# r9y9/deepvoice3_pytorch

Measured on NVIDIA H100. Metric: mel-frames/sec training step (B=16,T_mel=800), higher is better.
Workload: dtype f32 via split 16-bit pairs (fp16 pairs forward, bf16 pairs for gradients; 3 wgmma passes per product, fp32 accumulate)

## Files before the change

### deepvoice3_pytorch_b200/csrc/tc_common.cuh

```cuda
#pragma once
#include <cuda.h>
#include <cuda_bf16.h>
#include "common.cuh"

namespace dv3 {
namespace tc {

__device__ __forceinline__ uint32_t smem_u32(const void* p) { return (uint32_t)__cvta_generic_to_shared(p); }

__device__ __forceinline__ void mbar_init(uint64_t* bar, uint32_t count) {
    asm volatile("mbarrier.init.shared::cta.b64 [%0], %1;" ::"r"(smem_u32(bar)), "r"(count));
}
__device__ __forceinline__ void fence_barrier_init() {
    asm volatile("fence.mbarrier_init.release.cluster;" ::: "memory");
}
__device__ __forceinline__ void fence_proxy_async() {
    asm volatile("fence.proxy.async.shared::cta;" ::: "memory");
}
__device__ __forceinline__ void mbar_arrive_expect_tx(uint64_t* bar, uint32_t bytes) {
    asm volatile("mbarrier.arrive.expect_tx.shared::cta.b64 _, [%0], %1;" ::"r"(smem_u32(bar)), "r"(bytes)
                 : "memory");
}
__device__ __forceinline__ void mbar_arrive(uint64_t* bar) {
    asm volatile("mbarrier.arrive.shared::cta.b64 _, [%0];" ::"r"(smem_u32(bar)) : "memory");
}
__device__ __forceinline__ void mbar_wait(uint64_t* bar, uint32_t parity) {
    asm volatile(
        "{\n"
        ".reg .pred p;\n"
        "DV3_WAIT:\n"
        "mbarrier.try_wait.parity.shared::cta.b64 p, [%0], %1;\n"
        "@p bra DV3_DONE;\n"
        "bra DV3_WAIT;\n"
        "DV3_DONE:\n"
        "}\n" ::"r"(smem_u32(bar)),
        "r"(parity)
        : "memory");
}

__device__ __forceinline__ void tma_load_3d(void* smem_dst, const CUtensorMap* map, uint64_t* bar, int c0, int c1,
                                            int c2) {
    asm volatile(
        "cp.async.bulk.tensor.3d.shared::cluster.global.mbarrier::complete_tx::bytes [%0], [%1, {%3, %4, %5}], [%2];"
        ::"r"(smem_u32(smem_dst)), "l"(map), "r"(smem_u32(bar)), "r"(c0), "r"(c1), "r"(c2)
        : "memory");
}
__device__ __forceinline__ void prefetch_tmap(const CUtensorMap* map) {
    asm volatile("prefetch.tensormap [%0];" ::"l"(map) : "memory");
}
__device__ __forceinline__ void prefetch_l2(const void* p) {
    asm volatile("prefetch.global.L2 [%0];" ::"l"(p));
}
__device__ __forceinline__ void tma_store_3d(const CUtensorMap* map, const void* smem_src, int c0, int c1, int c2) {
    asm volatile("cp.async.bulk.tensor.3d.global.shared::cta.bulk_group [%0, {%2, %3, %4}], [%1];"
                 ::"l"(map), "r"(smem_u32(smem_src)), "r"(c0), "r"(c1), "r"(c2)
                 : "memory");
}
__device__ __forceinline__ void bulk_commit() { asm volatile("cp.async.bulk.commit_group;" ::: "memory"); }
__device__ __forceinline__ void bulk_wait_read() { asm volatile("cp.async.bulk.wait_group.read 0;" ::: "memory"); }
__device__ __forceinline__ void bulk_wait() { asm volatile("cp.async.bulk.wait_group 0;" ::: "memory"); }
__device__ __forceinline__ void mbar_arrive_cnt(uint64_t* bar, uint32_t count) {
    asm volatile("mbarrier.arrive.shared::cta.b64 _, [%0], %1;" ::"r"(smem_u32(bar)), "r"(count) : "memory");
}
__device__ __forceinline__ void named_bar_sync(int id, int threads) {
    asm volatile("bar.sync %0, %1;" ::"r"(id), "r"(threads) : "memory");
}

template <int N>
__device__ __forceinline__ void setmaxnreg_dec() { asm volatile("setmaxnreg.dec.sync.aligned.u32 %0;" ::"n"(N)); }
template <int N>
__device__ __forceinline__ void setmaxnreg_inc() { asm volatile("setmaxnreg.inc.sync.aligned.u32 %0;" ::"n"(N)); }

__device__ __forceinline__ void wgmma_fence() { asm volatile("wgmma.fence.sync.aligned;" ::: "memory"); }
__device__ __forceinline__ void wgmma_commit() { asm volatile("wgmma.commit_group.sync.aligned;" ::: "memory"); }
template <int N>
__device__ __forceinline__ void wgmma_wait() { asm volatile("wgmma.wait_group.sync.aligned %0;" ::"n"(N) : "memory"); }
__device__ __forceinline__ int frag_row(int i, int warp_in_wg, int lane) {
    return 16 * warp_in_wg + (lane >> 2) + 8 * ((i >> 1) & 1);
}
__device__ __forceinline__ int frag_col(int i, int lane) { return 8 * (i >> 2) + 2 * (lane & 3) + (i & 1); }

__device__ __forceinline__ uint64_t make_wgmma_desc(uint32_t saddr, uint32_t lbo, uint32_t sbo, uint32_t layout) {
    uint64_t d = 0;
    d |= (uint64_t)((saddr & 0x3FFFF) >> 4);
    d |= (uint64_t)((lbo >> 4) & 0x3FFF) << 16;
    d |= (uint64_t)((sbo >> 4) & 0x3FFF) << 32;
    d |= (uint64_t)layout << 62;
    return d;
}
constexpr uint32_t WG_SW128 = 1, WG_SW64 = 2;

template <int TA, int TB>
__device__ __forceinline__ void wgmma_f16_n64(float* d, uint64_t a, uint64_t b, uint32_t acc) {
    asm volatile(
        "{\n.reg .pred p;\nsetp.ne.b32 p, %34, 0;\n"
        "wgmma.mma_async.sync.aligned.m64n64k16.f32.f16.f16 {%0, %1, %2, %3, %4, %5, %6, %7, %8, %9, %10, %11, %12, %13, %14, %15, %16, %17, %18, %19, %20, %21, %22, %23, %24, %25, %26, %27, %28, %29, %30, %31}, %32, %33, p, 1, 1, %35, %36;\n}\n"
        : "+f"(d[0]), "+f"(d[1]), "+f"(d[2]), "+f"(d[3]), "+f"(d[4]), "+f"(d[5]), "+f"(d[6]), "+f"(d[7]), "+f"(d[8]), "+f"(d[9]), "+f"(d[10]), "+f"(d[11]), "+f"(d[12]), "+f"(d[13]), "+f"(d[14]), "+f"(d[15]), "+f"(d[16]), "+f"(d[17]), "+f"(d[18]), "+f"(d[19]), "+f"(d[20]), "+f"(d[21]), "+f"(d[22]), "+f"(d[23]), "+f"(d[24]), "+f"(d[25]), "+f"(d[26]), "+f"(d[27]), "+f"(d[28]), "+f"(d[29]), "+f"(d[30]), "+f"(d[31])
        : "l"(a), "l"(b), "r"(acc), "n"(TA), "n"(TB));
}
template <int TA, int TB>
__device__ __forceinline__ void wgmma_bf16_n64(float* d, uint64_t a, uint64_t b, uint32_t acc) {
    asm volatile(
        "{\n.reg .pred p;\nsetp.ne.b32 p, %34, 0;\n"
        "wgmma.mma_async.sync.aligned.m64n64k16.f32.bf16.bf16 {%0, %1, %2, %3, %4, %5, %6, %7, %8, %9, %10, %11, %12, %13, %14, %15, %16, %17, %18, %19, %20, %21, %22, %23, %24, %25, %26, %27, %28, %29, %30, %31}, %32, %33, p, 1, 1, %35, %36;\n}\n"
        : "+f"(d[0]), "+f"(d[1]), "+f"(d[2]), "+f"(d[3]), "+f"(d[4]), "+f"(d[5]), "+f"(d[6]), "+f"(d[7]), "+f"(d[8]), "+f"(d[9]), "+f"(d[10]), "+f"(d[11]), "+f"(d[12]), "+f"(d[13]), "+f"(d[14]), "+f"(d[15]), "+f"(d[16]), "+f"(d[17]), "+f"(d[18]), "+f"(d[19]), "+f"(d[20]), "+f"(d[21]), "+f"(d[22]), "+f"(d[23]), "+f"(d[24]), "+f"(d[25]), "+f"(d[26]), "+f"(d[27]), "+f"(d[28]), "+f"(d[29]), "+f"(d[30]), "+f"(d[31])
        : "l"(a), "l"(b), "r"(acc), "n"(TA), "n"(TB));
}
template <int TA, int TB>
__device__ __forceinline__ void wgmma_f16_n128(float* d, uint64_t a, uint64_t b, uint32_t acc) {
    asm volatile(
        "{\n.reg .pred p;\nsetp.ne.b32 p, %66, 0;\n"
        "wgmma.mma_async.sync.aligned.m64n128k16.f32.f16.f16 {%0, %1, %2, %3, %4, %5, %6, %7, %8, %9, %10, %11, %12, %13, %14, %15, %16, %17, %18, %19, %20, %21, %22, %23, %24, %25, %26, %27, %28, %29, %30, %31, %32, %33, %34, %35, %36, %37, %38, %39, %40, %41, %42, %43, %44, %45, %46, %47, %48, %49, %50, %51, %52, %53, %54, %55, %56, %57, %58, %59, %60, %61, %62, %63}, %64, %65, p, 1, 1, %67, %68;\n}\n"
        : "+f"(d[0]), "+f"(d[1]), "+f"(d[2]), "+f"(d[3]), "+f"(d[4]), "+f"(d[5]), "+f"(d[6]), "+f"(d[7]), "+f"(d[8]), "+f"(d[9]), "+f"(d[10]), "+f"(d[11]), "+f"(d[12]), "+f"(d[13]), "+f"(d[14]), "+f"(d[15]), "+f"(d[16]), "+f"(d[17]), "+f"(d[18]), "+f"(d[19]), "+f"(d[20]), "+f"(d[21]), "+f"(d[22]), "+f"(d[23]), "+f"(d[24]), "+f"(d[25]), "+f"(d[26]), "+f"(d[27]), "+f"(d[28]), "+f"(d[29]), "+f"(d[30]), "+f"(d[31]), "+f"(d[32]), "+f"(d[33]), "+f"(d[34]), "+f"(d[35]), "+f"(d[36]), "+f"(d[37]), "+f"(d[38]), "+f"(d[39]), "+f"(d[40]), "+f"(d[41]), "+f"(d[42]), "+f"(d[43]), "+f"(d[44]), "+f"(d[45]), "+f"(d[46]), "+f"(d[47]), "+f"(d[48]), "+f"(d[49]), "+f"(d[50]), "+f"(d[51]), "+f"(d[52]), "+f"(d[53]), "+f"(d[54]), "+f"(d[55]), "+f"(d[56]), "+f"(d[57]), "+f"(d[58]), "+f"(d[59]), "+f"(d[60]), "+f"(d[61]), "+f"(d[62]), "+f"(d[63])
        : "l"(a), "l"(b), "r"(acc), "n"(TA), "n"(TB));
}
template <int TA, int TB>
__device__ __forceinline__ void wgmma_bf16_n128(float* d, uint64_t a, uint64_t b, uint32_t acc) {
    asm volatile(
        "{\n.reg .pred p;\nsetp.ne.b32 p, %66, 0;\n"
        "wgmma.mma_async.sync.aligned.m64n128k16.f32.bf16.bf16 {%0, %1, %2, %3, %4, %5, %6, %7, %8, %9, %10, %11, %12, %13, %14, %15, %16, %17, %18, %19, %20, %21, %22, %23, %24, %25, %26, %27, %28, %29, %30, %31, %32, %33, %34, %35, %36, %37, %38, %39, %40, %41, %42, %43, %44, %45, %46, %47, %48, %49, %50, %51, %52, %53, %54, %55, %56, %57, %58, %59, %60, %61, %62, %63}, %64, %65, p, 1, 1, %67, %68;\n}\n"
        : "+f"(d[0]), "+f"(d[1]), "+f"(d[2]), "+f"(d[3]), "+f"(d[4]), "+f"(d[5]), "+f"(d[6]), "+f"(d[7]), "+f"(d[8]), "+f"(d[9]), "+f"(d[10]), "+f"(d[11]), "+f"(d[12]), "+f"(d[13]), "+f"(d[14]), "+f"(d[15]), "+f"(d[16]), "+f"(d[17]), "+f"(d[18]), "+f"(d[19]), "+f"(d[20]), "+f"(d[21]), "+f"(d[22]), "+f"(d[23]), "+f"(d[24]), "+f"(d[25]), "+f"(d[26]), "+f"(d[27]), "+f"(d[28]), "+f"(d[29]), "+f"(d[30]), "+f"(d[31]), "+f"(d[32]), "+f"(d[33]), "+f"(d[34]), "+f"(d[35]), "+f"(d[36]), "+f"(d[37]), "+f"(d[38]), "+f"(d[39]), "+f"(d[40]), "+f"(d[41]), "+f"(d[42]), "+f"(d[43]), "+f"(d[44]), "+f"(d[45]), "+f"(d[46]), "+f"(d[47]), "+f"(d[48]), "+f"(d[49]), "+f"(d[50]), "+f"(d[51]), "+f"(d[52]), "+f"(d[53]), "+f"(d[54]), "+f"(d[55]), "+f"(d[56]), "+f"(d[57]), "+f"(d[58]), "+f"(d[59]), "+f"(d[60]), "+f"(d[61]), "+f"(d[62]), "+f"(d[63])
        : "l"(a), "l"(b), "r"(acc), "n"(TA), "n"(TB));
}
template <int TA, int TB>
__device__ __forceinline__ void wgmma_f16_n256(float* d, uint64_t a, uint64_t b, uint32_t acc) {
    asm volatile(
        "{\n.reg .pred p;\nsetp.ne.b32 p, %130, 0;\n"
        "wgmma.mma_async.sync.aligned.m64n256k16.f32.f16.f16 {%0, %1, %2, %3, %4, %5, %6, %7, %8, %9, %10, %11, %12, %13, %14, %15, %16, %17, %18, %19, %20, %21, %22, %23, %24, %25, %26, %27, %28, %29, %30, %31, %32, %33, %34, %35, %36, %37, %38, %39, %40, %41, %42, %43, %44, %45, %46, %47, %48, %49, %50, %51, %52, %53, %54, %55, %56, %57, %58, %59, %60, %61, %62, %63, %64, %65, %66, %67, %68, %69, %70, %71, %72, %73, %74, %75, %76, %77, %78, %79, %80, %81, %82, %83, %84, %85, %86, %87, %88, %89, %90, %91, %92, %93, %94, %95, %96, %97, %98, %99, %100, %101, %102, %103, %104, %105, %106, %107, %108, %109, %110, %111, %112, %113, %114, %115, %116, %117, %118, %119, %120, %121, %122, %123, %124, %125, %126, %127}, %128, %129, p, 1, 1, %131, %132;\n}\n"
        : "+f"(d[0]), "+f"(d[1]), "+f"(d[2]), "+f"(d[3]), "+f"(d[4]), "+f"(d[5]), "+f"(d[6]), "+f"(d[7]), "+f"(d[8]), "+f"(d[9]), "+f"(d[10]), "+f"(d[11]), "+f"(d[12]), "+f"(d[13]), "+f"(d[14]), "+f"(d[15]), "+f"(d[16]), "+f"(d[17]), "+f"(d[18]), "+f"(d[19]), "+f"(d[20]), "+f"(d[21]), "+f"(d[22]), "+f"(d[23]), "+f"(d[24]), "+f"(d[25]), "+f"(d[26]), "+f"(d[27]), "+f"(d[28]), "+f"(d[29]), "+f"(d[30]), "+f"(d[31]), "+f"(d[32]), "+f"(d[33]), "+f"(d[34]), "+f"(d[35]), "+f"(d[36]), "+f"(d[37]), "+f"(d[38]), "+f"(d[39]), "+f"(d[40]), "+f"(d[41]), "+f"(d[42]), "+f"(d[43]), "+f"(d[44]), "+f"(d[45]), "+f"(d[46]), "+f"(d[47]), "+f"(d[48]), "+f"(d[49]), "+f"(d[50]), "+f"(d[51]), "+f"(d[52]), "+f"(d[53]), "+f"(d[54]), "+f"(d[55]), "+f"(d[56]), "+f"(d[57]), "+f"(d[58]), "+f"(d[59]), "+f"(d[60]), "+f"(d[61]), "+f"(d[62]), "+f"(d[63]), "+f"(d[64]), "+f"(d[65]), "+f"(d[66]), "+f"(d[67]), "+f"(d[68]), "+f"(d[69]), "+f"(d[70]), "+f"(d[71]), "+f"(d[72]), "+f"(d[73]), "+f"(d[74]), "+f"(d[75]), "+f"(d[76]), "+f"(d[77]), "+f"(d[78]), "+f"(d[79]), "+f"(d[80]), "+f"(d[81]), "+f"(d[82]), "+f"(d[83]), "+f"(d[84]), "+f"(d[85]), "+f"(d[86]), "+f"(d[87]), "+f"(d[88]), "+f"(d[89]), "+f"(d[90]), "+f"(d[91]), "+f"(d[92]), "+f"(d[93]), "+f"(d[94]), "+f"(d[95]), "+f"(d[96]), "+f"(d[97]), "+f"(d[98]), "+f"(d[99]), "+f"(d[100]), "+f"(d[101]), "+f"(d[102]), "+f"(d[103]), "+f"(d[104]), "+f"(d[105]), "+f"(d[106]), "+f"(d[107]), "+f"(d[108]), "+f"(d[109]), "+f"(d[110]), "+f"(d[111]), "+f"(d[112]), "+f"(d[113]), "+f"(d[114]), "+f"(d[115]), "+f"(d[116]), "+f"(d[117]), "+f"(d[118]), "+f"(d[119]), "+f"(d[120]), "+f"(d[121]), "+f"(d[122]), "+f"(d[123]), "+f"(d[124]), "+f"(d[125]), "+f"(d[126]), "+f"(d[127])
        : "l"(a), "l"(b), "r"(acc), "n"(TA), "n"(TB));
}
template <int TA, int TB>
__device__ __forceinline__ void wgmma_bf16_n256(float* d, uint64_t a, uint64_t b, uint32_t acc) {
    asm volatile(
        "{\n.reg .pred p;\nsetp.ne.b32 p, %130, 0;\n"
        "wgmma.mma_async.sync.aligned.m64n256k16.f32.bf16.bf16 {%0, %1, %2, %3, %4, %5, %6, %7, %8, %9, %10, %11, %12, %13, %14, %15, %16, %17, %18, %19, %20, %21, %22, %23, %24, %25, %26, %27, %28, %29, %30, %31, %32, %33, %34, %35, %36, %37, %38, %39, %40, %41, %42, %43, %44, %45, %46, %47, %48, %49, %50, %51, %52, %53, %54, %55, %56, %57, %58, %59, %60, %61, %62, %63, %64, %65, %66, %67, %68, %69, %70, %71, %72, %73, %74, %75, %76, %77, %78, %79, %80, %81, %82, %83, %84, %85, %86, %87, %88, %89, %90, %91, %92, %93, %94, %95, %96, %97, %98, %99, %100, %101, %102, %103, %104, %105, %106, %107, %108, %109, %110, %111, %112, %113, %114, %115, %116, %117, %118, %119, %120, %121, %122, %123, %124, %125, %126, %127}, %128, %129, p, 1, 1, %131, %132;\n}\n"
        : "+f"(d[0]), "+f"(d[1]), "+f"(d[2]), "+f"(d[3]), "+f"(d[4]), "+f"(d[5]), "+f"(d[6]), "+f"(d[7]), "+f"(d[8]), "+f"(d[9]), "+f"(d[10]), "+f"(d[11]), "+f"(d[12]), "+f"(d[13]), "+f"(d[14]), "+f"(d[15]), "+f"(d[16]), "+f"(d[17]), "+f"(d[18]), "+f"(d[19]), "+f"(d[20]), "+f"(d[21]), "+f"(d[22]), "+f"(d[23]), "+f"(d[24]), "+f"(d[25]), "+f"(d[26]), "+f"(d[27]), "+f"(d[28]), "+f"(d[29]), "+f"(d[30]), "+f"(d[31]), "+f"(d[32]), "+f"(d[33]), "+f"(d[34]), "+f"(d[35]), "+f"(d[36]), "+f"(d[37]), "+f"(d[38]), "+f"(d[39]), "+f"(d[40]), "+f"(d[41]), "+f"(d[42]), "+f"(d[43]), "+f"(d[44]), "+f"(d[45]), "+f"(d[46]), "+f"(d[47]), "+f"(d[48]), "+f"(d[49]), "+f"(d[50]), "+f"(d[51]), "+f"(d[52]), "+f"(d[53]), "+f"(d[54]), "+f"(d[55]), "+f"(d[56]), "+f"(d[57]), "+f"(d[58]), "+f"(d[59]), "+f"(d[60]), "+f"(d[61]), "+f"(d[62]), "+f"(d[63]), "+f"(d[64]), "+f"(d[65]), "+f"(d[66]), "+f"(d[67]), "+f"(d[68]), "+f"(d[69]), "+f"(d[70]), "+f"(d[71]), "+f"(d[72]), "+f"(d[73]), "+f"(d[74]), "+f"(d[75]), "+f"(d[76]), "+f"(d[77]), "+f"(d[78]), "+f"(d[79]), "+f"(d[80]), "+f"(d[81]), "+f"(d[82]), "+f"(d[83]), "+f"(d[84]), "+f"(d[85]), "+f"(d[86]), "+f"(d[87]), "+f"(d[88]), "+f"(d[89]), "+f"(d[90]), "+f"(d[91]), "+f"(d[92]), "+f"(d[93]), "+f"(d[94]), "+f"(d[95]), "+f"(d[96]), "+f"(d[97]), "+f"(d[98]), "+f"(d[99]), "+f"(d[100]), "+f"(d[101]), "+f"(d[102]), "+f"(d[103]), "+f"(d[104]), "+f"(d[105]), "+f"(d[106]), "+f"(d[107]), "+f"(d[108]), "+f"(d[109]), "+f"(d[110]), "+f"(d[111]), "+f"(d[112]), "+f"(d[113]), "+f"(d[114]), "+f"(d[115]), "+f"(d[116]), "+f"(d[117]), "+f"(d[118]), "+f"(d[119]), "+f"(d[120]), "+f"(d[121]), "+f"(d[122]), "+f"(d[123]), "+f"(d[124]), "+f"(d[125]), "+f"(d[126]), "+f"(d[127])
        : "l"(a), "l"(b), "r"(acc), "n"(TA), "n"(TB));
// ... 16 lines not shown
```

### deepvoice3_pytorch_b200/csrc/tc_gemm.cu

```cuda
#include "tc_common.cuh"
#include "tc_ring.cuh"
#include "../../include/dv3b200.h"

namespace dv3 {

using namespace tc;

constexpr int TC_CONV_THREADS = 512;
constexpr int TC_PRODUCER_REGS = 24;
constexpr int TC_CONSUMER_REGS = 168;
constexpr int TC_EPILOGUE_REGS = 152;
static_assert(TC_PRODUCER_REGS <= 65536 / TC_CONV_THREADS && TC_CONSUMER_REGS >= 65536 / TC_CONV_THREADS &&
              TC_EPILOGUE_REGS >= 65536 / TC_CONV_THREADS, "setmaxnreg direction of each warpgroup");
static_assert(128 * TC_PRODUCER_REGS + 256 * TC_CONSUMER_REGS + 128 * TC_EPILOGUE_REGS <= 65536, "register file");
constexpr int TC_EPILOGUE_LEAD = 3 * 128;
constexpr int TC_LAST_PARTS = 3;
constexpr int MAX_TAPS_TC = 8;
enum { TC_GATED = 0, TC_CONV = 1 };

struct TcMaps { CUtensorMap a[2]; CUtensorMap b[2]; };

struct TcParams {
    int T;
    int Nc;
// ... 205 lines not shown
    static_assert(Cfg::NCOLS <= 128, "main + cross accumulators must fit in the registers of a consumer thread");
    static_assert(Cfg::STAGES >= 2, "pipeline needs at least two stages");
    constexpr int STAGE = Cfg::STAGE, STAGES = Cfg::STAGES;
    constexpr int NR = Cfg::NCOLS / 2;
    pdl_trigger();
    extern __shared__ uint8_t smem_raw[];
    uint8_t* smem = smem_raw + ((1024 - (smem_u32(smem_raw) & 1023)) & 1023);
    float* acc_tile = reinterpret_cast<float*>(smem + STAGES * STAGE);
    uint64_t* full = reinterpret_cast<uint64_t*>(smem + STAGES * STAGE + Cfg::ACC_TILE + Cfg::STAGING);
    uint64_t* empty = full + STAGES;
    uint64_t* acc_full = empty + STAGES;
    uint64_t* acc_empty = acc_full + 1;
    uint64_t* in_full = acc_empty + 1;
    const int warp = threadIdx.x >> 5, lane = threadIdx.x & 31;

    if (threadIdx.x == 0) {
#pragma unroll
        for (int pl = 0; pl < NPL; ++pl) prefetch_tmap(&maps.a[pl]);
#pragma unroll
        for (int pl = 0; pl < NPL; ++pl) prefetch_tmap(&maps.b[pl]);
        for (int s = 0; s < STAGES; ++s) { mbar_init(&full[s], 1); mbar_init(&empty[s], 2); }
        mbar_init(acc_full, 256);
        mbar_init(acc_empty, 128);
        mbar_init(in_full, 1);
        fence_barrier_init();
    }
    __syncthreads();
    pdl_wait();

    if (warp >= 12) {
        setmaxnreg_inc<TC_EPILOGUE_REGS>();
        const Handoff h = {acc_tile, acc_tile + Cfg::ACC_TILE / 4, acc_empty, in_full};
        if (blockIdx.x < num_units) stage(decode(blockIdx.x), h);
        int n = 0;
        for (int u = blockIdx.x; u < num_units; u += gridDim.x, ++n) {
            const auto w = decode(u);
            const bool last = u + gridDim.x >= num_units;
            mbar_wait(acc_full, n & 1);
            if (last) epilogue(w, n, h, TC_LAST_PARTS - 1, TC_LAST_PARTS);
            else {
                epilogue(w, n, h, 0, 1);
                stage(decode(u + gridDim.x), h);
            }
        }
    } else if (warp >= 8) {
        setmaxnreg_dec<TC_PRODUCER_REGS>();
        if (warp == 8 && lane == 0) {
            int it = 0;
            for (int u = blockIdx.x; u < num_units; u += gridDim.x) {
                const auto w = decode(u);
                for (int kit = 0; kit < w.n_iters; ++kit, ++it) {
                    const int s = it % STAGES, ph = (it / STAGES) & 1;
                    mbar_wait(&empty[s], ph ^ 1);
                    mbar_arrive_expect_tx(&full[s], STAGE);
                    load(w, kit, smem + s * STAGE, &full[s]);
                }
            }
        }
    } else {
        setmaxnreg_inc<TC_CONSUMER_REGS>();
        const int wg = warp >> 2, wq = warp & 3;
        float acc[NR], xacc[NPL == 2 ? NR : 1];
        int it = 0, n = 0;
        for (int u = blockIdx.x; u < num_units; u += gridDim.x, ++n) {
            const auto w = decode(u);
#pragma unroll
            for (int i = 0; i < NR; ++i) {
                acc[i] = 0.f;
                if constexpr (NPL == 2) xacc[i] = 0.f;
            }
            for (int kit = 0; kit < w.n_iters; ++kit, ++it) {
                const int s = it % STAGES, ph = (it / STAGES) & 1;
                mbar_wait(&full[s], ph);
                wgmma_fence();
                mma(smem + s * STAGE, wg, acc, xacc);
                wgmma_commit();
                wgmma_wait<1>();
                if (kit > 0 && (threadIdx.x & 127) == 0) mbar_arrive(&empty[(it - 1) % STAGES]);
            }
            wgmma_wait<0>();
            if (w.n_iters > 0 && (threadIdx.x & 127) == 0) mbar_arrive(&empty[(it - 1) % STAGES]);
            const float gm = gmain(w);
            mbar_wait(acc_empty, (n & 1) ^ 1);
            const int sw = (((wq & 1) << 2) | (lane >> 4)) ^ ((lane & 3) << 1);
            float* const frag0 = Cfg::DENSE ? acc_tile + (2 * wg + (wq >> 1)) * Cfg::NCOLS * 32 + (lane & 3) * 64 +
                                                  ((lane >> 2) & 3)
                                            : acc_tile;
#pragma unroll
            for (int i = 0; i < NR; ++i) {
                float* dst = Cfg::DENSE
                    ? frag0 + (i >> 2) * 256 + (i & 1) * 32 + ((sw ^ (i & 3)) << 2)
                    : &acc_tile[(64 * wg + frag_row(i, wq, lane)) * Cfg::ACC_PITCH + frag_col(i, lane)];
                if constexpr (NPL == 2) *dst = fmaf(xacc[i], LO_INV, acc[i] * gm);
                else *dst = acc[i] * gm;
            }
            mbar_arrive(acc_full);
            if (u + gridDim.x >= num_units) {
                const Handoff h = {acc_tile, acc_tile + Cfg::ACC_TILE / 4, acc_empty, in_full};
                mbar_wait(acc_full, n & 1);
                epilogue(w, n, h, wg, TC_LAST_PARTS);
            }
        }
    }
}

template <int MODE, int NBOX, int BR, int BK, bool BF16, int NPL>
__global__ void __launch_bounds__(TC_CONV_THREADS, 1)
tc_conv_kernel(const __grid_constant__ TcMaps maps, const __grid_constant__ TcOutMaps om,
               const __grid_constant__ TcParams p, int tiles_x, int tiles_y, int num_tiles) {
    using Cfg = TcCfg<NBOX, BK, BR, NPL>;
    constexpr int NCOLS = Cfg::NCOLS;
    constexpr int TILE = 128 * BK * 2, TILE_B = BR * BK * 2;
    constexpr int B_OFF = NPL * TILE;
    constexpr int A_HALF = 64 * BK * 2;
    const int n_iters = p.k * p.kb_n;

    struct Tile { int a_row0, a_z, b_row0, b_row1, n_iters; };
    auto decode = [&](int tile) {
        Tile w;
        const int ty = tile % tiles_y, r = tile / tiles_y;
        w.a_z = r / tiles_x;
        w.a_row0 = (r % tiles_x) * 128;
        if (MODE == TC_GATED) { w.b_row0 = ty * BR; w.b_row1 = p.Nc + ty * BR; }
        else { w.b_row0 = ty * BR * NBOX; w.b_row1 = w.b_row0 + BR; }
        w.n_iters = n_iters;
        return w;
    };
    auto load = [&](const Tile& w, int kit, uint8_t* st, uint64_t* bar) {
        const int j = kit / p.kb_n, kb = kit - j * p.kb_n;
        const int ax = kb * BK, ay = w.a_row0 + p.tap_off[j];
        const int by0 = j * p.rows_per_tap + w.b_row0, by1 = j * p.rows_per_tap + w.b_row1;
#pragma unroll
        for (int pl = 0; pl < NPL; ++pl) {
            tma_load_3d(st + pl * TILE, &maps.a[pl], bar, ax, ay, w.a_z);
            uint8_t* bdst = st + B_OFF + pl * NBOX * TILE_B;
            tma_load_3d(bdst, &maps.b[pl], bar, ax, by0, 0);
            if (NBOX == 2) tma_load_3d(bdst + TILE_B, &maps.b[pl], bar, ax, by1, 0);
        }
    };
    auto mma = [&](const uint8_t* st, int wg, float* acc, float* xacc) {
        const uint32_t sa = smem_u32(st) + wg * A_HALF, sb = smem_u32(st + B_OFF);
#pragma unroll
        for (int kk = 0; kk < BK / 16; ++kk) {
            const uint32_t ko = kk * 32;
            const uint64_t a0 = make_desc<BK>(sa + ko), b0 = make_desc<BK>(sb + ko);
            wgmma_mma<NCOLS, 0, 0>(BF16, acc, a0, b0, 1);
            if constexpr (NPL == 2) {
                const uint64_t a1 = make_desc<BK>(sa + TILE + ko), b1 = make_desc<BK>(sb + NBOX * TILE_B + ko);
                wgmma_mma<NCOLS, 0, 0>(BF16, xacc, a0, b1, 1);
                wgmma_mma<NCOLS, 0, 0>(BF16, xacc, a1, b0, 1);
            }
        }
    };
    auto gmain = [&](const Tile&) { return p.gmain; };
    auto epilogue = [&](const Tile& w, int n, const Handoff& h, int part, int nparts) {
        if (MODE == TC_GATED) {
            if (nparts == 1) epilogue_gated<BR, 32>(p, om, h, n, w.a_row0, w.a_z, w.b_row0, 0, 1);
            else epilogue_gated<BR, BR / 8>(p, om, h, n, w.a_row0, w.a_z, w.b_row0, part, nparts);
        } else {
            if (nparts == 1) epilogue_conv<NCOLS, 32>(p, om, h, w.a_row0, w.a_z, w.b_row0, 0, 1);
            else epilogue_conv<NCOLS, NCOLS / 8>(p, om, h, w.a_row0, w.a_z, w.b_row0, part, nparts);
        }
    };
    auto stage = [&](const Tile& w, const Handoff& h) {
        if (MODE == TC_GATED) {
            stage_residual<BR>(p, om, h, w.a_row0, w.a_z, w.b_row0);
            if (p.spk) prefetch_bct(p.spk, p.T, p.Nc, w.a_z, w.b_row0, BR, w.a_row0);
        } else {
            if (p.addmode != 0) prefetch_bct(p.e1, p.T, p.Nc, w.a_z, w.b_row0, NCOLS, w.a_row0);
            if (p.addmode == 2) prefetch_bct(p.e2, p.T, p.Nc, w.a_z, w.b_row0, NCOLS, w.a_row0);
        }
    };
    tc_pipeline<Cfg, NPL>(maps, num_tiles, decode, load, mma, gmain, epilogue, stage);
}

struct TcMnParams {
    int T, B, Mw, Nw, k;
    int tap_off[MAX_TAPS_TC];
    int nsplit, batches_per_split, kb_n;
    int tiles_n, tiles_m, num_units;
    float* dw; long long split_stride;
    int msplit; long long s_m, s_mh, s_n, s_j;
    float gcoef;
};

template <int NPL>
__global__ void __launch_bounds__(TC_CONV_THREADS, 1)
tc_wgrad_mn_kernel(const __grid_constant__ TcMaps maps, const __grid_constant__ TcMnParams p) {
    using Cfg = WgCfg<NPL>;
    constexpr int A_PL = 2 * WG_BOX, B_PL = 2 * WG_BOX;
    constexpr uint32_t LBO = 4096, SBO = 1024;

    struct Unit { int m0, n0, j, s, b_beg, n_iters; };
    auto decode = [&](int u) {
        Unit w;
        w.n0 = (u % p.tiles_n) * 128;
        int r = u / p.tiles_n;
        w.m0 = (r % p.tiles_m) * 128;
        r /= p.tiles_m;
        w.j = r % p.k;
        w.s = r / p.k;
        w.b_beg = w.s * p.batches_per_split;
        const int b_end = min(p.B, w.b_beg + p.batches_per_split);
        w.n_iters = (b_end > w.b_beg ? b_end - w.b_beg : 0) * p.kb_n;
        return w;
    };
    auto load = [&](const Unit& w, int kit, uint8_t* st, uint64_t* bar) {
        const int bi = kit / p.kb_n, tc_ = kit - bi * p.kb_n;
        const int b = w.b_beg + bi, t0 = tc_ * 32;
#pragma unroll
        for (int pl = 0; pl < NPL; ++pl) {
#pragma unroll
            for (int h = 0; h < 2; ++h)
                tma_load_3d(st + pl * A_PL + h * WG_BOX, &maps.a[pl], bar, w.m0 + h * 64, t0, b);
#pragma unroll
            for (int q = 0; q < 2; ++q)
                tma_load_3d(st + NPL * A_PL + pl * B_PL + q * WG_BOX, &maps.b[pl], bar, w.n0 + q * 64,
                            t0 + p.tap_off[w.j], b);
        }
    };
    auto mma = [&](const uint8_t* st, int wg, float* acc, float* xacc) {
        const uint32_t sa = smem_u32(st);
#pragma unroll
        for (int kk = 0; kk < 2; ++kk) {
            const uint32_t ko = kk * 16 * 128;
            const uint64_t a0 = make_wgmma_desc(sa + wg * WG_BOX + ko, LBO, SBO, WG_SW128);
            const uint64_t b0 = make_wgmma_desc(sa + NPL * A_PL + ko, LBO, SBO, WG_SW128);
            wgmma_mma<128, 1, 1>(true, acc, a0, b0, 1);
            if constexpr (NPL == 2) {
                const uint64_t a1 = make_wgmma_desc(sa + A_PL + wg * WG_BOX + ko, LBO, SBO, WG_SW128);
                const uint64_t b1 = make_wgmma_desc(sa + 2 * A_PL + B_PL + ko, LBO, SBO, WG_SW128);
                wgmma_mma<128, 1, 1>(true, xacc, a0, b1, 1);
                wgmma_mma<128, 1, 1>(true, xacc, a1, b0, 1);
            }
        }
    };
    auto gmain = [&](const Unit& w) { return 1.f + p.gcoef * (float)(2 * w.n_iters); };
    auto epilogue = [&](const Unit& w, int, const Handoff& h, int part, int nparts) {
        const float* acc_tile = h.tile;
        const int r = threadIdx.x & 127;
        const int cw = nparts == 1 ? 128 : 16;
        float* __restrict__ out = p.dw + (size_t)w.s * p.split_stride + (size_t)w.j * p.s_j;
        const int rows = min(128, p.Mw - w.m0), cols = min(128, p.Nw - w.n0);
        if (p.s_n == 1) {
            if (r < cols) {
                float* __restrict__ o = out + w.n0 + r;
#pragma unroll 1
                for (int i0 = part * cw; i0 < rows; i0 += nparts * cw) {
                    const int i1 = min(i0 + cw, rows);
                    int mr = (w.m0 + i0) % p.msplit, mq = (w.m0 + i0) / p.msplit;
#pragma unroll 4
                    for (int i = i0; i < i1; ++i) {
                        o[(size_t)mr * p.s_m + (size_t)mq * p.s_mh] = acc_tile[i * Cfg::ACC_PITCH + r];
                        if (++mr == p.msplit) { mr = 0; ++mq; }
                    }
                }
            }
        } else if (r < rows) {
            const int m = w.m0 + r;
            float* __restrict__ o = out + (size_t)(m % p.msplit) * p.s_m + (size_t)(m / p.msplit) * p.s_mh +
                                    (size_t)w.n0 * p.s_n;
            const float* arow = acc_tile + r * Cfg::ACC_PITCH;
#pragma unroll 1
            for (int c0 = part * cw; c0 < cols; c0 += nparts * cw) {
                const int c1 = min(c0 + cw, cols);
#pragma unroll 4
                for (int c = c0; c < c1; ++c) o[(size_t)c * p.s_n] = arow[c];
            }
        }
        if (threadIdx.x >= TC_EPILOGUE_LEAD) mbar_arrive(h.acc_empty);
    };
    tc_pipeline<Cfg, NPL>(maps, p.num_units, decode, load, mma, gmain, epilogue, [](const Unit&, const Handoff&) {});
}

typedef CUresult (*EncodeTiledFn)(CUtensorMap*, CUtensorMapDataType, cuuint32_t, void*, const cuuint64_t*,
                                  const cuuint64_t*, const cuuint32_t*, const cuuint32_t*, CUtensorMapInterleave,
                                  CUtensorMapSwizzle, CUtensorMapL2promotion, CUtensorMapFloatOOBfill);

static EncodeTiledFn encode_fn() {
    static const EncodeTiledFn fn = [] {
        void* f = nullptr;
        cudaDriverEntryPointQueryResult qres;
        cudaError_t e = cudaGetDriverEntryPoint("cuTensorMapEncodeTiled", &f, cudaEnableDefault, &qres);
        return (e == cudaSuccess) ? (EncodeTiledFn)f : (EncodeTiledFn) nullptr;
    }();
    return fn;
}

int encode_tmap_bf16_3d(CUtensorMap* map, const void* base, uint64_t d0, uint64_t d1, uint64_t d2,
                        uint64_t stride1_bytes, uint64_t stride2_bytes, uint32_t box0, uint32_t box1) {
    const EncodeTiledFn enc = encode_fn();
    if (!enc) { set_error("cuTensorMapEncodeTiled entry point unavailable"); return 1; }
    cuuint64_t dims[3] = {d0, d1, d2};
    cuuint64_t strides[2] = {stride1_bytes, stride2_bytes};
    cuuint32_t box[3] = {box0, box1, 1};
    cuuint32_t estr[3] = {1, 1, 1};
    const CUtensorMapSwizzle sw = box0 * 2 == 128 ? CU_TENSOR_MAP_SWIZZLE_128B : CU_TENSOR_MAP_SWIZZLE_64B;
    CUresult r = enc(map, CU_TENSOR_MAP_DATA_TYPE_BFLOAT16, 3, const_cast<void*>(base), dims, strides, box, estr,
                     CU_TENSOR_MAP_INTERLEAVE_NONE, sw, CU_TENSOR_MAP_L2_PROMOTION_L2_256B,
                     CU_TENSOR_MAP_FLOAT_OOB_FILL_NONE);
    if (r != CUDA_SUCCESS) {
        set_error("cuTensorMapEncodeTiled failed (%d): dims=(%llu,%llu,%llu) strides=(%llu,%llu) box=(%u,%u)", (int)r,
                  (unsigned long long)d0, (unsigned long long)d1, (unsigned long long)d2,
                  (unsigned long long)stride1_bytes, (unsigned long long)stride2_bytes, box0, box1);
        return 1;
    }
    return 0;
}

static int encode_tmap_f32_bct(CUtensorMap* map, const float* base, int B, int Nc, int T, int box_c) {
    const EncodeTiledFn enc = encode_fn();
    if (!enc) { set_error("cuTensorMapEncodeTiled entry point unavailable"); return 1; }
    cuuint64_t dims[3] = {(cuuint64_t)T, (cuuint64_t)Nc, (cuuint64_t)B};
    cuuint64_t strides[2] = {(cuuint64_t)T * 4, (cuuint64_t)Nc * T * 4};
    cuuint32_t box[3] = {32, (cuuint32_t)box_c, 1};
    cuuint32_t estr[3] = {1, 1, 1};
    CUresult r = enc(map, CU_TENSOR_MAP_DATA_TYPE_FLOAT32, 3, const_cast<float*>(base), dims, strides, box, estr,
                     CU_TENSOR_MAP_INTERLEAVE_NONE, CU_TENSOR_MAP_SWIZZLE_128B, CU_TENSOR_MAP_L2_PROMOTION_L2_256B,
                     CU_TENSOR_MAP_FLOAT_OOB_FILL_NONE);
    if (r != CUDA_SUCCESS) {
        set_error("cuTensorMapEncodeTiled failed (%d): fp32 (B,C,T) = (%d,%d,%d) box=(32,%d)", (int)r, B, Nc, T, box_c);
        return 1;
    }
    return 0;
}

static bool tma_rows(const float* base, int T) { return T % 4 == 0 && ((uintptr_t)base & 15) == 0; }

template <typename K>
static int ensure_smem(K kern, int bytes, const char* what) {
    cudaError_t e = cudaFuncSetAttribute(kern, cudaFuncAttributeMaxDynamicSharedMemorySize, bytes);
    if (e != cudaSuccess) { set_error("%s: cannot set %d B dynamic smem: %s", what, bytes, cudaGetErrorString(e)); return 1; }
    return 0;
}

template <class Cfg, auto kern, typename... Args>
static int launch_persistent(int units, cudaStream_t st, const char* what, const Args&... args) {
    static const int configured = ensure_smem(kern, Cfg::SMEM, what);
    if (configured) return 1;
    const int sms = config().sms, grid = units < sms ? units : sms;
    cudaError_t e = launch_k(kern, dim3(grid), dim3(TC_CONV_THREADS), (size_t)Cfg::SMEM, st, args...);
    if (e != cudaSuccess) { set_error("%s: launch failed: %s", what, cudaGetErrorString(e)); return 1; }
    return check_launch(what);
}

template <int MODE, int NBOX, int BR, int BK, bool BF16, int NPL>
static int launch_conv_fmt(const TcMaps& maps, const TcOutMaps& om, const TcParams& p, int tiles_x, int tiles_y,
                           int batch, cudaStream_t st, const char* what) {
    const int num_tiles = tiles_x * tiles_y * batch;
    return launch_persistent<TcCfg<NBOX, BK, BR, NPL>, tc_conv_kernel<MODE, NBOX, BR, BK, BF16, NPL>>(
        num_tiles, st, what, maps, om, p, tiles_x, tiles_y, num_tiles);
}

template <int MODE, int NBOX, int BR, int BK, int NPL = 2>
static int launch_conv(const TcMaps& maps, const TcOutMaps& om, const TcParams& p, int tiles_x, int tiles_y, int batch,
                       cudaStream_t st, const char* what) {
    if (p.operand_bf16)
        return launch_conv_fmt<MODE, NBOX, BR, BK, true, NPL>(maps, om, p, tiles_x, tiles_y, batch, st, what);
    return launch_conv_fmt<MODE, NBOX, BR, BK, false, NPL>(maps, om, p, tiles_x, tiles_y, batch, st, what);
}

static void fill_taps_tc(int* tap_off, int k, int dilation, int causal, bool transpose) {
    const int padl = causal ? (k - 1) * dilation : (k - 1) / 2 * dilation;
    for (int j = 0; j < MAX_TAPS_TC; ++j)
        tap_off[j] = j < k ? (transpose ? (padl - j * dilation) : (j * dilation - padl)) : 0;
}

static inline const void* plane(const void* base, int pl, long long plane_elems) {
    return (const char*)base + (size_t)pl * plane_elems * 2;
}

}

using namespace dv3;

extern "C" {

int dv3_tc_supported(int B, int C, int T, int k) {
    return (C % 128 == 0) && T >= 1 && k >= 1 && k <= MAX_TAPS_TC && B >= 1 && B <= 65535;
}
int dv3_tc_conv_supported(int B, int Cin, int Cout, int T, int k) {
    return T >= 1 && k >= 1 && k <= MAX_TAPS_TC && B >= 1 && B <= 65535 && (k == 1 || Cout % 128 == 0) && Cin >= 8 &&
           Cout >= 1;
}

int dv3_tc_convblock_fwd(const void* xd, const void* w, int npl, const float* bias, const float* spk,
                         const float* res, float* y, float* save_a, float* save_s, int B, int C, int T, int k,
                         int dilation, int causal, int mode, int residual, const void* fuse, void* stream) {
    DV3_REQUIRE(dv3_tc_supported(B, C, T, k), "tc_convblock_fwd: unsupported shape B=%d C=%d T=%d k=%d", B, C, T, k);
    DV3_REQUIRE(npl == 1 || npl == 2, "tc_convblock_fwd: npl must be 1 or 2");
    DV3_REQUIRE(fuse == nullptr, "tc_convblock_fwd: fuse must be NULL");
    TcMaps maps;
    const int t_tiles = (T + 127) / 128;
    const int BK = npl == 2 ? 32 : 64;
    for (int pl = 0; pl < npl; ++pl) {
        if (encode_tmap_bf16_3d(&maps.a[pl], plane(xd, pl, (long long)B * T * C), C, T, B, (uint64_t)C * 2,
                                (uint64_t)T * C * 2, BK, 128)) return 1;
        if (encode_tmap_bf16_3d(&maps.b[pl], plane(w, pl, (long long)k * 2 * C * C), C, (uint64_t)k * 2 * C, 1,
                                (uint64_t)C * 2, (uint64_t)k * 2 * C * C * 2, BK, 64)) return 1;
    }
    TcParams p = {};
    p.T = T; p.Nc = C; p.rows_per_tap = 2 * C; p.k = k; p.kb_n = C / BK;
    fill_taps_tc(p.tap_off, k, dilation, causal, false);
    p.bias = bias; p.spk = spk; p.res = res; p.y = y; p.save_a = save_a; p.save_s = save_s;
    p.gate_mode = mode; p.residual = residual;
    p.gmain = 1.f + config().tc_gamma * (float)(p.k * p.kb_n * (BK / 16));
    const bool need_res = mode != 0 || residual;
// ... 31 lines not shown
    for (int pl = 0; pl < npl; ++pl) {
        if (encode_tmap_bf16_3d(&maps.a[pl], plane(a, pl, (long long)B * T * Kp), Kc, T, B, (uint64_t)Kp * 2,
                                (uint64_t)T * Kp * 2, bk, 128)) return 1;
        if (encode_tmap_bf16_3d(&maps.b[pl], plane(w, pl, (long long)k * Nc * Kp), Kc, (uint64_t)k * Nc, 1,
                                (uint64_t)Kp * 2, (uint64_t)k * Nc * Kp * 2, bk, br)) return 1;
    }
    TcParams p = {};
    p.T = T; p.Nc = Nc; p.rows_per_tap = Nc; p.k = k; p.kb_n = (Kc + bk - 1) / bk;
    fill_taps_tc(p.tap_off, k, dilation, causal, transpose_taps != 0);
    p.out = out; p.bias = bias; p.relu = relu; p.e1 = e1; p.e2 = e2; p.alpha = alpha; p.addmode = addmode;
    p.p_drop = p_drop; p.seed_ptr = seed_ptr; p.salt = salt;
    p.gmain = 1.f + config().tc_gamma * (float)(p.k * p.kb_n * (bk / 16));
    p.operand_bf16 = transpose_taps ? 1 : 0;
    TcOutMaps om = {};
    p.tma_out = tma_rows(out, T);
    if (p.tma_out && encode_tmap_f32_bct(&om.out[0], out, B, Nc, T, br)) return 1;
    const int tiles_y = (Nc + br - 1) / br;
    if (npl == 1) {
        if (narrow) {
            if (k64) return launch_conv<TC_CONV, 1, 64, 64, 1>(maps, om, p, t_tiles, tiles_y, B, st, "tc_conv(64)");
            return launch_conv<TC_CONV, 1, 64, 32, 1>(maps, om, p, t_tiles, tiles_y, B, st, "tc_conv(64,bk32)");
        }
        if (k64) return launch_conv<TC_CONV, 1, 128, 64, 1>(maps, om, p, t_tiles, tiles_y, B, st, "tc_conv(128,bk64)");
        return launch_conv<TC_CONV, 1, 128, 32, 1>(maps, om, p, t_tiles, tiles_y, B, st, "tc_conv(128)");
    }
    if (narrow) {
        if (k64) return launch_conv<TC_CONV, 1, 64, 64>(maps, om, p, t_tiles, tiles_y, B, st, "tc_conv(64)");
        return launch_conv<TC_CONV, 1, 64, 32>(maps, om, p, t_tiles, tiles_y, B, st, "tc_conv(64,bk32)");
    }
    return launch_conv<TC_CONV, 1, 128, 32>(maps, om, p, t_tiles, tiles_y, B, st, "tc_conv(128)");
}

constexpr double WG_UNIT_ITERS = 25.0;
constexpr double WG_SLAB_BYTES_PER_ITER = 1.5e6;
int dv3_tc_wgrad_nsplit(int B, int Mw, int Nw, int T, int k) {
    const long long tk = (long long)((Mw + 127) / 128) * ((Nw + 127) / 128) * k;
    const long long kb_n = (T + 31) / 32, sms = config().sms;
    const double slab = (double)Mw * Nw * k * 8.0 / WG_SLAB_BYTES_PER_ITER;
    auto cost = [&](int ns) {
        const long long bps = (B + ns - 1) / ns, U = tk * ns, U_full = tk * (ns - 1), G = U < sms ? U : sms;
        const long long L = bps * kb_n, L_last = (B - (ns - 1) * bps) * kb_n;
        return (double)((U_full + G - 1) / G) * (double)(L - L_last) +
               (double)((U + G - 1) / G) * ((double)L_last + WG_UNIT_ITERS) + ns * slab;
    };
    double best = 0.0;
    for (int bps = B, prev = 0; bps >= 1; --bps) {
        const int ns = (B + bps - 1) / bps;
        if (ns != prev && (prev == 0 || cost(ns) < best)) best = cost(ns);
        prev = ns;
    }
    for (int bps = B, prev = 0; bps >= 1; --bps) {
        const int ns = (B + bps - 1) / bps;
        if (ns != prev && cost(ns) <= 1.03 * best) return ns;
        prev = ns;
    }
    return 1;
}

int dv3_tc_wgrad_mn_npl(const void* dy, const void* xd, int npl, float* dw_partials, long long split_stride, int B,
                        int Mw, int Nw, int T, int k, int dilation, int causal, int msplit, long long s_m,
                        long long s_mh, long long s_n, long long s_j, void* stream) {
    DV3_REQUIRE(k >= 1 && k <= MAX_TAPS_TC && B <= 65535, "tc_wgrad_mn: unsupported shape k=%d", k);
    DV3_REQUIRE(npl == 1 || npl == 2, "tc_wgrad_mn: npl must be 1 or 2");
    const int Mp = (Mw + 7) / 8 * 8, Np = (Nw + 7) / 8 * 8;
    TcMaps maps;
    for (int pl = 0; pl < npl; ++pl) {
        if (encode_tmap_bf16_3d(&maps.a[pl], plane(dy, pl, (long long)B * T * Mp), Mw, T, B, (uint64_t)Mp * 2,
                                (uint64_t)T * Mp * 2, 64, 32)) return 1;
        if (encode_tmap_bf16_3d(&maps.b[pl], plane(xd, pl, (long long)B * T * Np), Nw, T, B, (uint64_t)Np * 2,
                                (uint64_t)T * Np * 2, 64, 32)) return 1;
    }
    TcMnParams p = {};
    p.T = T; p.B = B; p.Mw = Mw; p.Nw = Nw; p.k = k; p.kb_n = (T + 31) / 32;
    fill_taps_tc(p.tap_off, k, dilation, causal, false);
    p.nsplit = dv3_tc_wgrad_nsplit(B, Mw, Nw, T, k);
    p.batches_per_split = (B + p.nsplit - 1) / p.nsplit;
    p.tiles_n = (Nw + 127) / 128; p.tiles_m = (Mw + 127) / 128;
    const long long units = (long long)p.tiles_n * p.tiles_m * k * p.nsplit;
    DV3_REQUIRE(units < (1ll << 31), "tc_wgrad_mn: %lld work units", units);
    p.num_units = (int)units;
    p.dw = dw_partials; p.split_stride = split_stride;
    p.msplit = msplit; p.s_m = s_m; p.s_mh = s_mh; p.s_n = s_n; p.s_j = s_j;
    p.gcoef = config().tc_gamma;
    cudaStream_t st = (cudaStream_t)stream;
    if (npl == 1)
        return launch_persistent<WgCfg<1>, tc_wgrad_mn_kernel<1>>(p.num_units, st, "tc_wgrad_mn", maps, p);
    return launch_persistent<WgCfg<2>, tc_wgrad_mn_kernel<2>>(p.num_units, st, "tc_wgrad_mn", maps, p);
}

int dv3_tc_wgrad_mn(const void* dy, const void* xd, float* dw_partials, long long split_stride, int B, int Mw,
                    int Nw, int T, int k, int dilation, int causal, int msplit, long long s_m, long long s_mh,
                    long long s_n, long long s_j, void* stream) {
    return dv3_tc_wgrad_mn_npl(dy, xd, 2, dw_partials, split_stride, B, Mw, Nw, T, k, dilation, causal, msplit, s_m,
                               s_mh, s_n, s_j, stream);
}

}
```

### deepvoice3_pytorch_b200/csrc/tc_ring.cuh

```cuda
#pragma once

namespace dv3 {

constexpr int SMEM_LIMIT = 232448;
constexpr int RING_SLACK = 1024 + 512;

template <int STAGE_BYTES, int TILE_COLS, int DEPTH, bool DENSE_TILE = false, int STAGING_BYTES = 0>
struct RingCfg {
    static constexpr int STAGE = STAGE_BYTES;
    static constexpr int NCOLS = TILE_COLS;
    static constexpr bool DENSE = DENSE_TILE;
    static constexpr int ACC_PITCH = DENSE ? NCOLS : NCOLS + 1;
    static constexpr int ACC_TILE = 128 * ACC_PITCH * 4;
    static constexpr int STAGING = STAGING_BYTES;
    static constexpr int STAGES = DEPTH;
    static constexpr int SMEM = STAGES * STAGE + ACC_TILE + STAGING + RING_SLACK;
    static constexpr int MAX_STAGES = (SMEM_LIMIT - ACC_TILE - STAGING - RING_SLACK) / STAGE;
    static_assert(STAGE % 1024 == 0, "ring stages keep the 1 KB alignment of the swizzled TMA tiles");
    static_assert(ACC_TILE % 1024 == 0 || !DENSE, "the dense tile and the staging buffer are swizzled TMA boxes");
    static_assert(STAGES >= 2, "pipeline needs at least two stages");
    static_assert(SMEM <= SMEM_LIMIT, "ring + hand-off tile + staging + barriers exceed the 227 KB of a CTA");
};

template <int NBOX, int BK, int BR, int NPL> struct ConvRing;
template <> struct ConvRing<2, 32, 64, 2> { static constexpr int STAGES = 4; };
template <> struct ConvRing<1, 32, 128, 2> { static constexpr int STAGES = 4; };
template <> struct ConvRing<1, 64, 64, 2> { static constexpr int STAGES = 4; };
template <> struct ConvRing<1, 32, 64, 2> { static constexpr int STAGES = 6; };
template <> struct ConvRing<2, 64, 64, 1> { static constexpr int STAGES = 4; };
template <> struct ConvRing<1, 64, 128, 1> { static constexpr int STAGES = 4; };
template <> struct ConvRing<1, 32, 128, 1> { static constexpr int STAGES = 6; };
template <> struct ConvRing<1, 64, 64, 1> { static constexpr int STAGES = 6; };
template <> struct ConvRing<1, 32, 64, 1> { static constexpr int STAGES = 6; };

template <int NBOX, int BK, int BR, int NPL = 2>
using TcCfg = RingCfg<NPL * (128 + NBOX * BR) * BK * 2, BR * NBOX, ConvRing<NBOX, BK, BR, NPL>::STAGES, true,
                      NBOX == 2 ? 128 * BR * 4 : 0>;

constexpr int WG_BOX = 64 * 32 * 2;
template <int NPL>
using WgCfg = RingCfg<NPL * 4 * WG_BOX, 128, NPL == 2 ? 5 : 6>;

}
```

Baseline: 1.754 million.

## Store weight-gradient partials via swizzled hand-off tile and TMA bulk stores

```diff
diff --git a/deepvoice3_pytorch_b200/csrc/tc_common.cuh b/deepvoice3_pytorch_b200/csrc/tc_common.cuh
--- a/deepvoice3_pytorch_b200/csrc/tc_common.cuh
+++ b/deepvoice3_pytorch_b200/csrc/tc_common.cuh
@@ -54,6 +54,12 @@
 __device__ __forceinline__ void tma_store_3d(const CUtensorMap* map, const void* smem_src, int c0, int c1, int c2) {
     asm volatile("cp.async.bulk.tensor.3d.global.shared::cta.bulk_group [%0, {%2, %3, %4}], [%1];"
                  ::"l"(map), "r"(smem_u32(smem_src)), "r"(c0), "r"(c1), "r"(c2)
+                 : "memory");
+}
+__device__ __forceinline__ void tma_store_4d(const CUtensorMap* map, const void* smem_src, int c0, int c1, int c2,
+                                             int c3) {
+    asm volatile("cp.async.bulk.tensor.4d.global.shared::cta.bulk_group [%0, {%2, %3, %4, %5}], [%1];"
+                 ::"l"(map), "r"(smem_u32(smem_src)), "r"(c0), "r"(c1), "r"(c2), "r"(c3)
                  : "memory");
 }
 __device__ __forceinline__ void bulk_commit() { asm volatile("cp.async.bulk.commit_group;" ::: "memory"); }
diff --git a/deepvoice3_pytorch_b200/csrc/tc_gemm.cu b/deepvoice3_pytorch_b200/csrc/tc_gemm.cu
--- a/deepvoice3_pytorch_b200/csrc/tc_gemm.cu
+++ b/deepvoice3_pytorch_b200/csrc/tc_gemm.cu
@@ -311,17 +311,33 @@
             if (w.n_iters > 0 && (threadIdx.x & 127) == 0) mbar_arrive(&empty[(it - 1) % STAGES]);
             const float gm = gmain(w);
             mbar_wait(acc_empty, (n & 1) ^ 1);
-            const int sw = (((wq & 1) << 2) | (lane >> 4)) ^ ((lane & 3) << 1);
-            float* const frag0 = Cfg::DENSE ? acc_tile + (2 * wg + (wq >> 1)) * Cfg::NCOLS * 32 + (lane & 3) * 64 +
-                                                  ((lane >> 2) & 3)
-                                            : acc_tile;
-#pragma unroll
-            for (int i = 0; i < NR; ++i) {
-                float* dst = Cfg::DENSE
-                    ? frag0 + (i >> 2) * 256 + (i & 1) * 32 + ((sw ^ (i & 3)) << 2)
-                    : &acc_tile[(64 * wg + frag_row(i, wq, lane)) * Cfg::ACC_PITCH + frag_col(i, lane)];
-                if constexpr (NPL == 2) *dst = fmaf(xacc[i], LO_INV, acc[i] * gm);
-                else *dst = acc[i] * gm;
+            auto handoff = [&](int i) {
+                if constexpr (NPL == 2) return fmaf(xacc[i], LO_INV, acc[i] * gm);
+                else return acc[i] * gm;
+            };
+            if constexpr (Cfg::TILE == TILE_ROWS_INNER) {
+                const int sw = (((wq & 1) << 2) | (lane >> 4)) ^ ((lane & 3) << 1);
+                float* const frag0 = acc_tile + (2 * wg + (wq >> 1)) * Cfg::NCOLS * 32 + (lane & 3) * 64 +
+                                     ((lane >> 2) & 3);
+#pragma unroll
+                for (int i = 0; i < NR; ++i) frag0[(i >> 2) * 256 + (i & 1) * 32 + ((sw ^ (i & 3)) << 2)] = handoff(i);
+            } else {
+                const int r8 = lane >> 2, odd = r8 & 1;
+                const int sw = ((lane >> 1) & 1) ^ r8 ^ (odd << 2);
+                float* const row0 = acc_tile + (64 * wg + 16 * wq + r8) * 32 + 2 * (lane & 1);
+                auto at = [&](int i) {
+                    return reinterpret_cast<float2*>(row0 + (i >> 4) * 4096 + ((i >> 1) & 1) * 256 +
+                                                     (((((i >> 2) & 3) << 1) ^ sw) << 2));
+                };
+#pragma unroll
+                for (int i = 0; i < NR; i += 2) {
+                    if (i & 8) continue;
+                    const float2 x = make_float2(handoff(i), handoff(i + 1));
+                    const float2 y = make_float2(handoff(i + 8), handoff(i + 9));
+                    *at(i) = odd ? y : x;
+                    *at(i + 8) = odd ? x : y;
+                }
+                fence_proxy_async();
             }
             mbar_arrive(acc_full);
             if (u + gridDim.x >= num_units) {
@@ -411,11 +427,13 @@
     float* dw; long long split_stride;
     int msplit; long long s_m, s_mh, s_n, s_j;
     float gcoef;
+    int tma_out;
 };
 
 template <int NPL>
 __global__ void __launch_bounds__(TC_CONV_THREADS, 1)
-tc_wgrad_mn_kernel(const __grid_constant__ TcMaps maps, const __grid_constant__ TcMnParams p) {
+tc_wgrad_mn_kernel(const __grid_constant__ TcMaps maps, const __grid_constant__ CUtensorMap out_map,
+                   const __grid_constant__ TcMnParams p) {
     using Cfg = WgCfg<NPL>;
     constexpr int A_PL = 2 * WG_BOX, B_PL = 2 * WG_BOX;
     constexpr uint32_t LBO = 4096, SBO = 1024;
@@ -467,6 +485,17 @@
     auto gmain = [&](const Unit& w) { return 1.f + p.gcoef * (float)(2 * w.n_iters); };
     auto epilogue = [&](const Unit& w, int, const Handoff& h, int part, int nparts) {
         const float* acc_tile = h.tile;
+        if (p.tma_out) {
+            if (threadIdx.x == TC_EPILOGUE_LEAD) {
+#pragma unroll
+                for (int q = 0; q < 4; ++q) {
+                    if (w.n0 + 32 * q >= p.Nw) break;
+                    tma_store_4d(&out_map, acc_tile + q * 4096, w.n0 + 32 * q, w.m0, w.j, w.s);
+                }
+            }
+            release_tile(h, true);
+            return;
+        }
         const int r = threadIdx.x & 127;
         const int cw = nparts == 1 ? 128 : 16;
         float* __restrict__ out = p.dw + (size_t)w.s * p.split_stride + (size_t)w.j * p.s_j;
@@ -474,13 +503,15 @@
         if (p.s_n == 1) {
             if (r < cols) {
                 float* __restrict__ o = out + w.n0 + r;
+                const float* col = acc_tile + (r >> 5) * 4096 + (r & 3);
+                const int cr = (r >> 2) & 7;
 #pragma unroll 1
                 for (int i0 = part * cw; i0 < rows; i0 += nparts * cw) {
                     const int i1 = min(i0 + cw, rows);
                     int mr = (w.m0 + i0) % p.msplit, mq = (w.m0 + i0) / p.msplit;
 #pragma unroll 4
                     for (int i = i0; i < i1; ++i) {
-                        o[(size_t)mr * p.s_m + (size_t)mq * p.s_mh] = acc_tile[i * Cfg::ACC_PITCH + r];
+                        o[(size_t)mr * p.s_m + (size_t)mq * p.s_mh] = col[i * 32 + ((cr ^ (i & 7)) << 2)];
                         if (++mr == p.msplit) { mr = 0; ++mq; }
                     }
                 }
@@ -489,15 +520,22 @@
             const int m = w.m0 + r;
             float* __restrict__ o = out + (size_t)(m % p.msplit) * p.s_m + (size_t)(m / p.msplit) * p.s_mh +
                                     (size_t)w.n0 * p.s_n;
-            const float* arow = acc_tile + r * Cfg::ACC_PITCH;
+            const float* row = acc_tile + r * 32;
 #pragma unroll 1
             for (int c0 = part * cw; c0 < cols; c0 += nparts * cw) {
                 const int c1 = min(c0 + cw, cols);
-#pragma unroll 4
-                for (int c = c0; c < c1; ++c) o[(size_t)c * p.s_n] = arow[c];
-            }
-        }
-        if (threadIdx.x >= TC_EPILOGUE_LEAD) mbar_arrive(h.acc_empty);
+#pragma unroll 2
+                for (int c = c0; c < c1; c += 4) {
+                    const float4 v = *reinterpret_cast<const float4*>(row + (c >> 5) * 4096 +
+                                                                      ((((c >> 2) & 7) ^ (r & 7)) << 2));
+                    o[(size_t)c * p.s_n] = v.x;
+                    if (c + 1 < c1) o[(size_t)(c + 1) * p.s_n] = v.y;
+                    if (c + 2 < c1) o[(size_t)(c + 2) * p.s_n] = v.z;
+                    if (c + 3 < c1) o[(size_t)(c + 3) * p.s_n] = v.w;
+                }
+            }
+        }
+        release_tile(h, false);
     };
     tc_pipeline<Cfg, NPL>(maps, p.num_units, decode, load, mma, gmain, epilogue, [](const Unit&, const Handoff&) {});
 }
@@ -552,6 +590,33 @@
         return 1;
     }
     return 0;
+}
+
+static int encode_tmap_f32_wgrad(CUtensorMap* map, float* base, int Mw, int Nw, int k, int nsplit, long long s_m,
+                                 long long s_j, long long split_stride) {
+    const EncodeTiledFn enc = encode_fn();
+    if (!enc) { set_error("cuTensorMapEncodeTiled entry point unavailable"); return 1; }
+    const cuuint64_t sj = k > 1 ? (cuuint64_t)s_j * 4 : (cuuint64_t)s_m * 4 * Mw;
+    cuuint64_t dims[4] = {(cuuint64_t)Nw, (cuuint64_t)Mw, (cuuint64_t)k, (cuuint64_t)nsplit};
+    cuuint64_t strides[3] = {(cuuint64_t)s_m * 4, sj, nsplit > 1 ? (cuuint64_t)split_stride * 4 : sj * k};
+    cuuint32_t box[4] = {32, 128, 1, 1};
+    cuuint32_t estr[4] = {1, 1, 1, 1};
+    CUresult r = enc(map, CU_TENSOR_MAP_DATA_TYPE_FLOAT32, 4, base, dims, strides, box, estr,
+                     CU_TENSOR_MAP_INTERLEAVE_NONE, CU_TENSOR_MAP_SWIZZLE_128B, CU_TENSOR_MAP_L2_PROMOTION_L2_256B,
+                     CU_TENSOR_MAP_FLOAT_OOB_FILL_NONE);
+    if (r != CUDA_SUCCESS) {
+        set_error("cuTensorMapEncodeTiled failed (%d): fp32 partials (Nw,Mw,k,nsplit) = (%d,%d,%d,%d) strides=(%lld,"
+                  "%lld,%lld)", (int)r, Nw, Mw, k, nsplit, s_m, s_j, split_stride);
+        return 1;
+    }
+    return 0;
+}
+
+static bool tma_partials(const float* base, int Mw, int k, int nsplit, int msplit, long long s_m, long long s_n,
+                         long long s_j, long long split_stride) {
+    auto a16 = [](long long s) { return s > 0 && s % 4 == 0; };
+    return s_n == 1 && msplit >= Mw && ((uintptr_t)base & 15) == 0 && a16(s_m) && (k == 1 || a16(s_j)) &&
+           (nsplit == 1 || a16(split_stride));
 }
 
 static bool tma_rows(const float* base, int T) { return T % 4 == 0 && ((uintptr_t)base & 15) == 0; }
@@ -749,10 +814,14 @@
     p.dw = dw_partials; p.split_stride = split_stride;
     p.msplit = msplit; p.s_m = s_m; p.s_mh = s_mh; p.s_n = s_n; p.s_j = s_j;
     p.gcoef = config().tc_gamma;
+    CUtensorMap out_map = {};
+    p.tma_out = tma_partials(dw_partials, Mw, k, p.nsplit, msplit, s_m, s_n, s_j, split_stride);
+    if (p.tma_out && encode_tmap_f32_wgrad(&out_map, dw_partials, Mw, Nw, k, p.nsplit, s_m, s_j, split_stride))
+        return 1;
     cudaStream_t st = (cudaStream_t)stream;
     if (npl == 1)
-        return launch_persistent<WgCfg<1>, tc_wgrad_mn_kernel<1>>(p.num_units, st, "tc_wgrad_mn", maps, p);
-    return launch_persistent<WgCfg<2>, tc_wgrad_mn_kernel<2>>(p.num_units, st, "tc_wgrad_mn", maps, p);
+        return launch_persistent<WgCfg<1>, tc_wgrad_mn_kernel<1>>(p.num_units, st, "tc_wgrad_mn", maps, out_map, p);
+    return launch_persistent<WgCfg<2>, tc_wgrad_mn_kernel<2>>(p.num_units, st, "tc_wgrad_mn", maps, out_map, p);
 }
 
 int dv3_tc_wgrad_mn(const void* dy, const void* xd, float* dw_partials, long long split_stride, int B, int Mw,
diff --git a/deepvoice3_pytorch_b200/csrc/tc_ring.cuh b/deepvoice3_pytorch_b200/csrc/tc_ring.cuh
--- a/deepvoice3_pytorch_b200/csrc/tc_ring.cuh
+++ b/deepvoice3_pytorch_b200/csrc/tc_ring.cuh
@@ -5,19 +5,20 @@
 constexpr int SMEM_LIMIT = 232448;
 constexpr int RING_SLACK = 1024 + 512;
 
-template <int STAGE_BYTES, int TILE_COLS, int DEPTH, bool DENSE_TILE = false, int STAGING_BYTES = 0>
+enum TileLayout { TILE_ROWS_INNER, TILE_COLS_INNER };
+template <int STAGE_BYTES, int TILE_COLS, int DEPTH, TileLayout LAYOUT, int STAGING_BYTES = 0>
 struct RingCfg {
     static constexpr int STAGE = STAGE_BYTES;
     static constexpr int NCOLS = TILE_COLS;
-    static constexpr bool DENSE = DENSE_TILE;
-    static constexpr int ACC_PITCH = DENSE ? NCOLS : NCOLS + 1;
-    static constexpr int ACC_TILE = 128 * ACC_PITCH * 4;
+    static constexpr TileLayout TILE = LAYOUT;
+    static constexpr int ACC_TILE = 128 * NCOLS * 4;
     static constexpr int STAGING = STAGING_BYTES;
     static constexpr int STAGES = DEPTH;
     static constexpr int SMEM = STAGES * STAGE + ACC_TILE + STAGING + RING_SLACK;
     static constexpr int MAX_STAGES = (SMEM_LIMIT - ACC_TILE - STAGING - RING_SLACK) / STAGE;
     static_assert(STAGE % 1024 == 0, "ring stages keep the 1 KB alignment of the swizzled TMA tiles");
-    static_assert(ACC_TILE % 1024 == 0 || !DENSE, "the dense tile and the staging buffer are swizzled TMA boxes");
+    static_assert(ACC_TILE % 1024 == 0, "the hand-off tile and the staging buffer are swizzled TMA boxes");
+    static_assert(LAYOUT == TILE_ROWS_INNER || NCOLS == 128, "column boxes of 32 columns x 128 rows");
     static_assert(STAGES >= 2, "pipeline needs at least two stages");
     static_assert(SMEM <= SMEM_LIMIT, "ring + hand-off tile + staging + barriers exceed the 227 KB of a CTA");
 };
@@ -34,11 +35,11 @@
 template <> struct ConvRing<1, 32, 64, 1> { static constexpr int STAGES = 6; };
 
 template <int NBOX, int BK, int BR, int NPL = 2>
-using TcCfg = RingCfg<NPL * (128 + NBOX * BR) * BK * 2, BR * NBOX, ConvRing<NBOX, BK, BR, NPL>::STAGES, true,
-                      NBOX == 2 ? 128 * BR * 4 : 0>;
+using TcCfg = RingCfg<NPL * (128 + NBOX * BR) * BK * 2, BR * NBOX, ConvRing<NBOX, BK, BR, NPL>::STAGES,
+                      TILE_ROWS_INNER, NBOX == 2 ? 128 * BR * 4 : 0>;
 
 constexpr int WG_BOX = 64 * 32 * 2;
 template <int NPL>
-using WgCfg = RingCfg<NPL * 4 * WG_BOX, 128, NPL == 2 ? 5 : 6>;
+using WgCfg = RingCfg<NPL * 4 * WG_BOX, 128, NPL == 2 ? 5 : 6, TILE_COLS_INNER>;
 
 }
```

Result: faster. 1.773 million, median of 6 (+1.1%).
